# LordLiang/DrawingSpinUp

Hardware: AMD Instinct MI355X
Metric: drawings/sec end-to-end (512x512, 6 views, 24 frames) (higher is better)
Workload: dtype f16 (diffusion) / f16 table + f32 MLP (NSR) / f32 (stage-1 deformable convolutions, IS-Net, contour) / f32 with bf16 x 3 products (stage-2 convolutions; the reference: cuDNN TF32)

## Files before the change

drawingspinup_amd/csrc/mesh_decimate_gpu.hip:

```cpp
#include "common.h"

#include <math.h>
#include <stdint.h>

#include <hipcub/hipcub.hpp>

namespace {

struct D3 {
  double x, y, z;
};
__device__ inline D3 operator+(D3 a, D3 b) { return {a.x + b.x, a.y + b.y, a.z + b.z}; }
__device__ inline D3 operator-(D3 a, D3 b) { return {a.x - b.x, a.y - b.y, a.z - b.z}; }
__device__ inline D3 operator*(D3 a, double s) { return {a.x * s, a.y * s, a.z * s}; }
__device__ inline double dot3(D3 a, D3 b) { return a.x * b.x + a.y * b.y + a.z * b.z; }
__device__ inline D3 cross3(D3 a, D3 b) {
  return {a.y * b.z - a.z * b.y, a.z * b.x - a.x * b.z, a.x * b.y - a.y * b.x};
}
__device__ inline double norm3(D3 a) { return sqrt(dot3(a, a)); }

struct Quad {
  double q[10];
};
__device__ inline void quad_zero(Quad& a) {
  for (int i = 0; i < 10; ++i) a.q[i] = 0.0;
}
__device__ inline void quad_add_plane(Quad& a, D3 n, double d, double w) {
  a.q[0] += w * n.x * n.x; a.q[1] += w * n.x * n.y; a.q[2] += w * n.x * n.z;
  a.q[3] += w * n.y * n.y; a.q[4] += w * n.y * n.z; a.q[5] += w * n.z * n.z;
  a.q[6] += w * n.x * d; a.q[7] += w * n.y * d; a.q[8] += w * n.z * d;
  a.q[9] += w * d * d;
}
__device__ inline double quad_eval(const Quad& a, D3 v) {
  return v.x * (a.q[0] * v.x + 2 * a.q[1] * v.y + 2 * a.q[2] * v.z) +
         v.y * (a.q[3] * v.y + 2 * a.q[4] * v.z) + a.q[5] * v.z * v.z +
         2 * (a.q[6] * v.x + a.q[7] * v.y + a.q[8] * v.z) + a.q[9];
}
struct Row4 {
  double c[4];
};
__device__ inline void row_swap_if(Row4& a, Row4& b, bool s) {
  if (s) { const Row4 t = a; a = b; b = t; }
}
__device__ inline void row_eliminate(Row4& r, const Row4& piv, int col) {
  const double f = r.c[col] / piv.c[col];
  for (int k = 0; k < 4; ++k) r.c[k] -= f * piv.c[k];
}
__device__ inline bool quad_minimum(const Quad& a, D3 o, D3& out) {
  const double a00 = a.q[0], a01 = a.q[1], a02 = a.q[2], a11 = a.q[3], a12 = a.q[4], a22 = a.q[5];
  const double b0 = a.q[6], b1 = a.q[7], b2 = a.q[8];
  const double c00 = a11 * a22 - a12 * a12, c01 = a02 * a12 - a01 * a22, c02 = a01 * a12 - a02 * a11;
  const double det = a00 * c00 + a01 * c01 + a02 * c02;
  const double tr = a00 + a11 + a22;
  if (!(tr > 0.0) || !(fabs(det) > 1e-9 * tr * tr * tr)) return false;
  Row4 r0 = {{a00, a01, a02, -(b0 + (a00 * o.x + a01 * o.y + a02 * o.z))}};
  Row4 r1 = {{a01, a11, a12, -(b1 + (a01 * o.x + a11 * o.y + a12 * o.z))}};
  Row4 r2 = {{a02, a12, a22, -(b2 + (a02 * o.x + a12 * o.y + a22 * o.z))}};
  row_swap_if(r0, r1, fabs(r1.c[0]) > fabs(r0.c[0]));
  row_swap_if(r0, r2, fabs(r2.c[0]) > fabs(r0.c[0]));
  if (!(fabs(r0.c[0]) > 0.0)) return false;
  row_eliminate(r1, r0, 0);
  row_eliminate(r2, r0, 0);
  row_swap_if(r1, r2, fabs(r2.c[1]) > fabs(r1.c[1]));
  if (!(fabs(r1.c[1]) > 0.0)) return false;
  row_eliminate(r2, r1, 1);
  if (!(fabs(r2.c[2]) > 0.0)) return false;
  const double z = r2.c[3] / r2.c[2];
  const double y = (r1.c[3] - r1.c[2] * z) / r1.c[1];
  const double x = (r0.c[3] - r0.c[1] * y - r0.c[2] * z) / r0.c[0];
  out = {o.x + x, o.y + y, o.z + z};
  return true;
}

struct Mesh {
  double* P;
  double* Q;
  int32_t* F;
  int32_t* voff;
  int32_t* vfaces;
  int64_t nv, nf;
};

__device__ inline D3 ldP(const Mesh& m, int32_t v) { return {m.P[3 * v], m.P[3 * v + 1], m.P[3 * v + 2]}; }
__device__ inline Quad ldQ(const Mesh& m, int32_t v) {
  Quad a;
  for (int i = 0; i < 10; ++i) a.q[i] = m.Q[10 * (int64_t)v + i];
  return a;
}
__device__ inline bool tri_has(const Mesh& m, int32_t t, int32_t v) {
  return m.F[3 * t] == v || m.F[3 * t + 1] == v || m.F[3 * t + 2] == v;
}

__device__ inline void edge_target(const Mesh& m, int32_t v0, int32_t v1, double& cost, D3& vbar) {
  Quad q = ldQ(m, v0);
  const Quad q1 = ldQ(m, v1);
  for (int i = 0; i < 10; ++i) q.q[i] += q1.q[i];
  const D3 p0 = ldP(m, v0), p1 = ldP(m, v1);
  const D3 mid = (p0 + p1) * 0.5;
  if (quad_minimum(q, mid, vbar)) {
    const double len = norm3(p1 - p0);
    if (norm3(vbar - mid) <= 4.0 * len) {
      cost = quad_eval(q, vbar);
      return;
    }
  }
  const D3 cand[3] = {p0, p1, (p0 + p1) * 0.5};
  cost = quad_eval(q, cand[0]);
  vbar = cand[0];
  for (int i = 1; i < 3; ++i) {
    const double c = quad_eval(q, cand[i]);
    if (c < cost) { cost = c; vbar = cand[i]; }
  }
}

__global__ void flag_nondegenerate_kernel(const int32_t* F, int64_t nf, uint8_t* flag) {
  for (int64_t t = blockIdx.x * (int64_t)blockDim.x + threadIdx.x; t < nf; t += (int64_t)gridDim.x * blockDim.x) {
    const int32_t a = F[3 * t], b = F[3 * t + 1], c = F[3 * t + 2];
    flag[t] = (a != b && b != c && a != c) ? 1 : 0;
  }
}

__global__ void degree_kernel(const int32_t* F, int64_t nf, int32_t* deg) {
  for (int64_t i = blockIdx.x * (int64_t)blockDim.x + threadIdx.x; i < 3 * nf; i += (int64_t)gridDim.x * blockDim.x)
    atomicAdd(&deg[F[i]], 1);
}

__global__ void fill_kernel(const int32_t* F, int64_t nf, const int32_t* voff, int32_t* cursor, int32_t* vfaces) {
  for (int64_t i = blockIdx.x * (int64_t)blockDim.x + threadIdx.x; i < 3 * nf; i += (int64_t)gridDim.x * blockDim.x) {
    const int32_t v = F[i];
    vfaces[voff[v] + atomicAdd(&cursor[v], 1)] = (int32_t)(i / 3);
  }
}

__global__ void sort_lists_kernel(const int32_t* voff, int32_t* vfaces, int64_t nv) {
  for (int64_t v = blockIdx.x * (int64_t)blockDim.x + threadIdx.x; v < nv; v += (int64_t)gridDim.x * blockDim.x) {
    const int32_t b = voff[v], e = voff[v + 1];
    for (int32_t i = b + 1; i < e; ++i) {
      const int32_t x = vfaces[i];
      int32_t j = i - 1;
      while (j >= b && vfaces[j] > x) { vfaces[j + 1] = vfaces[j]; --j; }
      vfaces[j + 1] = x;
    }
  }
}

__device__ inline bool has_half_edge(const Mesh& m, int32_t a, int32_t b) {
  for (int32_t i = m.voff[a]; i < m.voff[a + 1]; ++i) {
    const int32_t t = m.vfaces[i];
    for (int k = 0; k < 3; ++k)
      if (m.F[3 * t + k] == a && m.F[3 * t + (k + 1) % 3] == b) return true;
  }
  return false;
}

__global__ void init_quadrics_kernel(Mesh m, double boundary_weight) {
  for (int64_t v = blockIdx.x * (int64_t)blockDim.x + threadIdx.x; v < m.nv; v += (int64_t)gridDim.x * blockDim.x) {
    Quad q;
    quad_zero(q);
    for (int32_t i = m.voff[v]; i < m.voff[v + 1]; ++i) {
      const int32_t t = m.vfaces[i];
      const int32_t a = m.F[3 * t], b = m.F[3 * t + 1], c = m.F[3 * t + 2];
      const D3 pa = ldP(m, a), pb = ldP(m, b), pc = ldP(m, c);
      const D3 cr = cross3(pb - pa, pc - pa);
      const double l = norm3(cr);
      if (!(l > 0.0)) continue;
      const D3 n = cr * (1.0 / l);
      quad_add_plane(q, n, -dot3(n, pa), 0.5 * l);
      if (boundary_weight > 0.0) {
        for (int k = 0; k < 3; ++k) {
          const int32_t e0 = m.F[3 * t + k], e1 = m.F[3 * t + (k + 1) % 3];
          if (e0 != (int32_t)v && e1 != (int32_t)v) continue;
          if (has_half_edge(m, e1, e0)) continue;
          int same = 0;
          for (int32_t j = m.voff[e0]; j < m.voff[e0 + 1]; ++j) {
            const int32_t t2 = m.vfaces[j];
            for (int kk = 0; kk < 3; ++kk)
              if (m.F[3 * t2 + kk] == e0 && m.F[3 * t2 + (kk + 1) % 3] == e1) ++same;
          }
          if (same != 1) continue;
          const int32_t lo = e0 < e1 ? e0 : e1, hi = e0 < e1 ? e1 : e0;
          D3 en = cross3(ldP(m, hi) - ldP(m, lo), n);
          const double el = norm3(en);
          if (!(el > 0.0)) continue;
          en = en * (1.0 / el);
          quad_add_plane(q, en, -dot3(en, ldP(m, lo)), boundary_weight * 0.5 * l);
        }
      }
    }
    for (int i = 0; i < 10; ++i) m.Q[10 * v + i] = q.q[i];
  }
}

__global__ void owner_flags_kernel(Mesh m, uint8_t* flag) {
  for (int64_t i = blockIdx.x * (int64_t)blockDim.x + threadIdx.x; i < 3 * m.nf; i += (int64_t)gridDim.x * blockDim.x) {
    const int64_t t = i / 3;
    const int k = (int)(i % 3);
    const int32_t a = m.F[3 * t + k], b = m.F[3 * t + (k + 1) % 3];
    flag[i] = (a < b || (a > b && !has_half_edge(m, b, a))) ? 1 : 0;
  }
}

typedef unsigned long long Reject;

__device__ inline unsigned long long ekey(int32_t a, int32_t b) {
  const uint32_t lo = a < b ? a : b, hi = a < b ? b : a;
  return ((unsigned long long)lo << 32) | hi;
}
__device__ inline unsigned long long mix64(unsigned long long k) {
  k ^= k >> 33; k *= 0xff51afd7ed558ccdull; k ^= k >> 33; k *= 0xc4ceb9fe1a85ec53ull; k ^= k >> 33;
  return k;
}
__device__ inline uint32_t slot_of(unsigned long long key, uint32_t n_slots) {
  return (uint32_t)(mix64(key) % n_slots);
}
__device__ inline unsigned long long reject_tag(unsigned long long key, uint32_t ver0, uint32_t ver1) {
  return mix64(key ^ mix64(((unsigned long long)ver0 << 32) | ver1)) & 0xffffffffffffull;
}

__global__ void edge_cost_kernel(Mesh m, const int32_t* edges, int64_t ne, const Reject* rej, uint32_t n_slots,
                                 const uint32_t* vver, uint32_t* cost_bits, uint32_t* edge_idx) {
  for (int64_t e = blockIdx.x * (int64_t)blockDim.x + threadIdx.x; e < ne; e += (int64_t)gridDim.x * blockDim.x) {
    const int32_t h = edges[e];
    const int32_t t = h / 3, k = h % 3;
    const int32_t a = m.F[3 * t + k], b = m.F[3 * t + (k + 1) % 3];
    const int32_t v0 = a < b ? a : b, v1 = a < b ? b : a;
    double cost; D3 vb;
    edge_target(m, v0, v1, cost, vb);
    float c = (float)(cost > 0.0 ? cost : 0.0);
    const unsigned long long key = ekey(v0, v1);
    if ((rej[slot_of(key, n_slots)] & 0xffffffffffffull) == reject_tag(key, vver[v0], vver[v1])) c = INFINITY;
    cost_bits[e] = __float_as_uint(c);
    edge_idx[e] = (uint32_t)e;
  }
}

__device__ inline void edge_ends(const Mesh& m, int32_t h, int32_t& v0, int32_t& v1) {
  const int32_t t = h / 3, k = h % 3;
  const int32_t a = m.F[3 * t + k], b = m.F[3 * t + (k + 1) % 3];
  v0 = a < b ? a : b;
  v1 = a < b ? b : a;
}

__device__ inline unsigned long long priority_of(int32_t v0, int32_t v1, uint32_t round, uint32_t r) {
  unsigned long long k = ekey(v0, v1) ^ ((unsigned long long)round * 0x9e3779b97f4a7c15ull);
  k ^= k >> 31; k *= 0xbf58476d1ce4e5b9ull; k ^= k >> 29; k *= 0x94d049bb133111ebull; k ^= k >> 32;
  return (k << 32) | r;
}

__device__ inline bool is_dirty(const Mesh& m, int32_t v0, int32_t v1, const uint32_t* touched, uint32_t round) {
  for (int pass = 0; pass < 2; ++pass) {
    const int32_t v = pass ? v1 : v0;
    for (int32_t i = m.voff[v]; i < m.voff[v + 1]; ++i) {
      const int32_t t = m.vfaces[i];
      for (int k = 0; k < 3; ++k)
        if (touched[m.F[3 * t + k]] == round) return true;
    }
  }
  return touched[v0] == round || touched[v1] == round;
}

__global__ void claim_kernel(Mesh m, const int32_t* edges, const uint32_t* sorted_idx, const uint32_t* sorted_cost,
                             int64_t ncand, uint32_t round, uint32_t seed, const uint32_t* touched,
                             const Reject* rej, uint32_t n_slots, const uint32_t* vver,
                             unsigned long long* claim) {
  for (int64_t r = blockIdx.x * (int64_t)blockDim.x + threadIdx.x; r < ncand; r += (int64_t)gridDim.x * blockDim.x) {
    if (sorted_cost[r] == 0x7f800000u) continue;
    int32_t v0, v1;
    edge_ends(m, edges[sorted_idx[r]], v0, v1);
    if (is_dirty(m, v0, v1, touched, round)) continue;
    {
      const unsigned long long key = ekey(v0, v1);
      if ((rej[slot_of(key, n_slots)] & 0xffffffffffffull) == reject_tag(key, vver[v0], vver[v1])) continue;
    }
    const unsigned long long pr = priority_of(v0, v1, seed, (uint32_t)r);
    for (int pass = 0; pass < 2; ++pass) {
      const int32_t v = pass ? v1 : v0;
      for (int32_t i = m.voff[v]; i < m.voff[v + 1]; ++i) {
        const int32_t t = m.vfaces[i];
        for (int k = 0; k < 3; ++k) atomicMin(&claim[m.F[3 * t + k]], pr);
      }
    }
  }
}

__global__ void collapse_kernel(Mesh m, const int32_t* edges, const uint32_t* sorted_idx, const uint32_t* sorted_cost,
                                int64_t ncand, uint32_t round, uint32_t seed, const unsigned long long* claim,
                                int link_test, uint8_t* f_alive, Reject* rej, uint32_t n_slots, uint32_t* vver,
                                uint32_t* touched_next, const uint32_t* touched, int32_t* counters) {
  for (int64_t r = blockIdx.x * (int64_t)blockDim.x + threadIdx.x; r < ncand; r += (int64_t)gridDim.x * blockDim.x) {
    if (sorted_cost[r] == 0x7f800000u) continue;
    int32_t v0, v1;
    edge_ends(m, edges[sorted_idx[r]], v0, v1);
    const unsigned long long pr = priority_of(v0, v1, seed, (uint32_t)r);
    if (claim[v0] != pr || claim[v1] != pr) continue;
    if (is_dirty(m, v0, v1, touched, round)) continue;
    double cost; D3 vbar;
    edge_target(m, v0, v1, cost, vbar);
    const int32_t b0 = m.voff[v0], e0 = m.voff[v0 + 1], b1 = m.voff[v1], e1 = m.voff[v1 + 1];
    int shared = 0;
    bool bad = false;
    for (int pass = 0; pass < 2 && !bad; ++pass) {
      const int32_t mv = pass ? v0 : v1, other = pass ? v1 : v0;
      for (int32_t i = m.voff[mv]; i < m.voff[mv + 1]; ++i) {
        const int32_t t = m.vfaces[i];
        if (tri_has(m, t, other)) { if (!pass) ++shared; continue; }
        D3 p[3], q[3];
        for (int k = 0; k < 3; ++k) {
          p[k] = ldP(m, m.F[3 * t + k]);
          q[k] = m.F[3 * t + k] == mv ? vbar : p[k];
        }
        const D3 before = cross3(p[1] - p[0], p[2] - p[0]);
        const D3 after = cross3(q[1] - q[0], q[2] - q[0]);
        if (dot3(before, after) < 0.0) { bad = true; break; }
      }
    }
    if (!bad && shared == 0) bad = true;
    if (!bad && link_test) {
      int common = 0;
      for (int32_t i = b0; i < e0; ++i) {
        const int32_t t = m.vfaces[i];
        for (int k = 0; k < 3; ++k) {
          const int32_t u = m.F[3 * t + k];
          if (u == v0 || u == v1) continue;
          bool first = true;
          for (int32_t j = b0; j < i && first; ++j)
            if (tri_has(m, m.vfaces[j], u)) first = false;
          if (first)
            for (int kk = 0; kk < k; ++kk)
              if (m.F[3 * t + kk] == u) first = false;
          if (!first) continue;
          bool in1 = false;
          for (int32_t j = b1; j < e1 && !in1; ++j)
            if (tri_has(m, m.vfaces[j], u)) in1 = true;
          if (in1) ++common;
        }
      }
      if (common != shared) bad = true;
      for (int32_t j = b1; j < e1 && !bad; ++j) {
        const int32_t t1 = m.vfaces[j];
        if (tri_has(m, t1, v0)) continue;
        int32_t xy[2], k2 = 0;
        for (int k = 0; k < 3; ++k)
          if (m.F[3 * t1 + k] != v1 && k2 < 2) xy[k2++] = m.F[3 * t1 + k];
        if (k2 < 2) continue;
        for (int32_t i = b0; i < e0; ++i) {
          const int32_t t0 = m.vfaces[i];
          if (!tri_has(m, t0, v1) && tri_has(m, t0, xy[0]) && tri_has(m, t0, xy[1])) { bad = true; break; }
        }
      }
    }
    if (bad) {
      const unsigned long long key = ekey(v0, v1);
      atomicMax(&rej[slot_of(key, n_slots)],
                ((unsigned long long)(round & 0xffffu) << 48) | reject_tag(key, vver[v0], vver[v1]));
      atomicAdd(&counters[1], 1);
      continue;
    }
    for (int pass = 0; pass < 2; ++pass) {
      const int32_t v = pass ? v1 : v0;
      for (int32_t i = m.voff[v]; i < m.voff[v + 1]; ++i) {
        const int32_t t = m.vfaces[i];
        for (int k = 0; k < 3; ++k) atomicAdd(&vver[m.F[3 * t + k]], 1u);
      }
    }
    int removed = 0;
    for (int32_t j = b1; j < e1; ++j) {
      const int32_t t = m.vfaces[j];
      if (tri_has(m, t, v0)) {
        f_alive[t] = 0;
        ++removed;
      } else {
        for (int k = 0; k < 3; ++k)
          if (m.F[3 * t + k] == v1) m.F[3 * t + k] = v0;
      }
    }
    m.P[3 * v0] = vbar.x; m.P[3 * v0 + 1] = vbar.y; m.P[3 * v0 + 2] = vbar.z;
    for (int i = 0; i < 10; ++i) m.Q[10 * (int64_t)v0 + i] += m.Q[10 * (int64_t)v1 + i];
    touched_next[v0] = round;
    touched_next[v1] = round;
    atomicAdd(&counters[0], 1);
    atomicAdd(&counters[2], removed);
  }
}

struct Tri {
  int32_t a, b, c;
};

inline size_t align256(size_t x) { return (x + 255) & ~(size_t)255; }

struct Layout {
  size_t off_Q, off_F2, off_voff, off_cursor, off_vfaces, off_flag, off_edges, off_iota, off_cost, off_cost2,
      off_idx, off_idx2, off_claim, off_vver, off_touched, off_touched2, off_rej, off_counters, off_nsel, off_cub, cub_bytes, total;
  uint32_t n_slots;
};

Layout make_layout(int64_t nv, int64_t nf) {
  Layout L;
  size_t o = 0;
  auto take = [&](size_t bytes) { size_t r = o; o += align256(bytes); return r; };
  L.off_Q = take((size_t)nv * 10 * sizeof(double));
  L.off_F2 = take((size_t)nf * 3 * sizeof(int32_t));
  L.off_voff = take((size_t)(nv + 1) * sizeof(int32_t));
  L.off_cursor = take((size_t)(nv + 1) * sizeof(int32_t));
  L.off_vfaces = take((size_t)nf * 3 * sizeof(int32_t));
  L.off_flag = take((size_t)nf * 3);
  L.off_edges = take((size_t)nf * 3 * sizeof(int32_t));
  L.off_iota = take((size_t)nf * 3 * sizeof(int32_t));
  L.off_cost = take((size_t)nf * 3 * sizeof(uint32_t));
  L.off_cost2 = take((size_t)nf * 3 * sizeof(uint32_t));
  L.off_idx = take((size_t)nf * 3 * sizeof(uint32_t));
  L.off_idx2 = take((size_t)nf * 3 * sizeof(uint32_t));
  L.off_claim = take((size_t)nv * sizeof(unsigned long long));
  L.off_vver = take((size_t)nv * sizeof(uint32_t));
  L.off_touched = take((size_t)nv * sizeof(uint32_t));
  L.off_touched2 = take((size_t)nv * sizeof(uint32_t));
  L.n_slots = (uint32_t)(nv * 2 + 1024);
  L.off_rej = take((size_t)L.n_slots * sizeof(Reject));
  L.off_counters = take(64);
  L.off_nsel = take(64);
  size_t b_scan = 0, b_sel_i = 0, b_sel_t = 0, b_sort = 0;
  hipcub::DeviceScan::ExclusiveSum(nullptr, b_scan, (int32_t*)nullptr, (int32_t*)nullptr, (int)(nv + 1));
  hipcub::DeviceSelect::Flagged(nullptr, b_sel_i, (int32_t*)nullptr, (uint8_t*)nullptr, (int32_t*)nullptr,
                                (int32_t*)nullptr, (int)(3 * nf));
  hipcub::DeviceSelect::Flagged(nullptr, b_sel_t, (Tri*)nullptr, (uint8_t*)nullptr, (Tri*)nullptr, (int32_t*)nullptr,
                                (int)nf);
  hipcub::DeviceRadixSort::SortPairs(nullptr, b_sort, (uint32_t*)nullptr, (uint32_t*)nullptr, (uint32_t*)nullptr,
                                     (uint32_t*)nullptr, (int)(3 * nf));
  L.cub_bytes = std::max(std::max(b_scan, b_sel_i), std::max(b_sel_t, b_sort)) + 256;
  L.off_cub = take(L.cub_bytes);
  L.total = o;
  return L;
}

__global__ void iota_kernel(int32_t* p, int64_t n) {
  for (int64_t i = blockIdx.x * (int64_t)blockDim.x + threadIdx.x; i < n; i += (int64_t)gridDim.x * blockDim.x) p[i] = (int32_t)i;
}

}

#define DSU_HIP_TRY(expr)                       \
  do {                                          \
    if ((expr) != hipSuccess) return DSU_ELAUNCH; \
  } while (0)

extern "C" {

int64_t dsu_mesh_decimate_parallel_workspace_bytes(int64_t n_verts, int64_t n_faces) {
  if (n_verts < 0 || n_faces < 0 || n_verts > (1 << 30) || n_faces > (1 << 29)) return DSU_EINVAL;
  return (int64_t)make_layout(n_verts, n_faces).total;
}

int dsu_mesh_decimate_parallel(double* verts, int64_t n_verts, int32_t* faces, int64_t n_faces,
                               int64_t stop_faces, int64_t floor_faces, double boundary_weight, int32_t flags,
                               int32_t max_rounds, double* out_quadrics, int64_t* out_n_faces,
                               int32_t* out_stats, void* workspace, int64_t workspace_bytes, void* stream) {
  if (n_verts < 0 || n_faces < 0 || stop_faces < floor_faces || floor_faces < 0 || !out_n_faces ||
      (n_verts && !verts) || (n_faces && !faces) || !(boundary_weight >= 0.0) || max_rounds < 0 ||
      n_verts > (1 << 30) || n_faces > (1 << 29))
    return DSU_EINVAL;
  hipStream_t s = (hipStream_t)stream;
  if (out_stats) out_stats[0] = out_stats[1] = out_stats[2] = 0;
  *out_n_faces = n_faces;
  if (n_faces == 0 || n_verts == 0) return DSU_OK;
  const Layout L = make_layout(n_verts, n_faces);
  if (!workspace || workspace_bytes < (int64_t)L.total) return DSU_EINVAL;
  char* w = (char*)workspace;
  double* Q = (double*)(w + L.off_Q);
  int32_t* F2 = (int32_t*)(w + L.off_F2);
  int32_t* voff = (int32_t*)(w + L.off_voff);
  int32_t* cursor = (int32_t*)(w + L.off_cursor);
  int32_t* vfaces = (int32_t*)(w + L.off_vfaces);
  uint8_t* flag = (uint8_t*)(w + L.off_flag);
  int32_t* edges = (int32_t*)(w + L.off_edges);
  int32_t* iota = (int32_t*)(w + L.off_iota);
  uint32_t* cost = (uint32_t*)(w + L.off_cost);
  uint32_t* cost2 = (uint32_t*)(w + L.off_cost2);
  uint32_t* idx = (uint32_t*)(w + L.off_idx);
  uint32_t* idx2 = (uint32_t*)(w + L.off_idx2);
  unsigned long long* claim = (unsigned long long*)(w + L.off_claim);
  uint32_t* vver = (uint32_t*)(w + L.off_vver);
  uint32_t* touched = (uint32_t*)(w + L.off_touched);
  uint32_t* touched2 = (uint32_t*)(w + L.off_touched2);
  Reject* rej = (Reject*)(w + L.off_rej);
  int32_t* counters = (int32_t*)(w + L.off_counters);
  int32_t* nsel = (int32_t*)(w + L.off_nsel);
  void* cub = (void*)(w + L.off_cub);
  const int T = 256;
  const int PASSES = 4;
  const int link_test = !(flags & 1);

  int32_t* F = faces;
  int64_t nf = n_faces;
  int32_t host_n = 0;
  auto compact_faces = [&]() -> int {
    size_t b = L.cub_bytes;
    if (hipcub::DeviceSelect::Flagged(cub, b, (Tri*)F, flag, (Tri*)F2, nsel, (int)nf, s) != hipSuccess)
      return DSU_ELAUNCH;
    if (hipMemcpyAsync(&host_n, nsel, sizeof(int32_t), hipMemcpyDeviceToHost, s) != hipSuccess) return DSU_ELAUNCH;
    if (hipStreamSynchronize(s) != hipSuccess) return DSU_ELAUNCH;
    nf = host_n;
    if (nf && hipMemcpyAsync(F, F2, (size_t)nf * 3 * sizeof(int32_t), hipMemcpyDeviceToDevice, s) != hipSuccess)
      return DSU_ELAUNCH;
    return DSU_OK;
  };
  auto build_csr = [&]() -> int {
    DSU_HIP_TRY(hipMemsetAsync(cursor, 0, (size_t)(n_verts + 1) * sizeof(int32_t), s));
    degree_kernel<<<dsu_capped_blocks(3 * nf, T), T, 0, s>>>(F, nf, cursor);
    size_t b = L.cub_bytes;
    if (hipcub::DeviceScan::ExclusiveSum(cub, b, cursor, voff, (int)(n_verts + 1), s) != hipSuccess)
      return DSU_ELAUNCH;
    DSU_HIP_TRY(hipMemsetAsync(cursor, 0, (size_t)(n_verts + 1) * sizeof(int32_t), s));
    fill_kernel<<<dsu_capped_blocks(3 * nf, T), T, 0, s>>>(F, nf, voff, cursor, vfaces);
    sort_lists_kernel<<<dsu_capped_blocks(n_verts, T), T, 0, s>>>(voff, vfaces, n_verts);
    DSU_CHECK_LAUNCH();
    return DSU_OK;
  };

  flag_nondegenerate_kernel<<<dsu_capped_blocks(nf, T), T, 0, s>>>(F, nf, flag);
  DSU_CHECK_LAUNCH();
  int rc = compact_faces();
  if (rc) return rc;
  DSU_HIP_TRY(hipMemsetAsync(vver, 0, (size_t)n_verts * sizeof(uint32_t), s));
  DSU_HIP_TRY(hipMemsetAsync(touched, 0xff, (size_t)n_verts * sizeof(uint32_t), s));
  DSU_HIP_TRY(hipMemsetAsync(touched2, 0xff, (size_t)n_verts * sizeof(uint32_t), s));
  DSU_HIP_TRY(hipMemsetAsync(rej, 0, (size_t)L.n_slots * sizeof(Reject), s));
  iota_kernel<<<dsu_capped_blocks(3 * nf, T), T, 0, s>>>(iota, 3 * nf);
  if ((rc = build_csr())) return rc;
  Mesh m{verts, Q, F, voff, vfaces, n_verts, nf};
  init_quadrics_kernel<<<dsu_capped_blocks(n_verts, T), T, 0, s>>>(m, boundary_weight);
  DSU_CHECK_LAUNCH();

  int rounds = 0, applied_total = 0, rejected_total = 0, stall = 0;
  while (nf > stop_faces && rounds < max_rounds) {
    const int64_t budget = (nf - floor_faces) / 2;
    if (budget < 1) break;
    m.nf = nf;
    owner_flags_kernel<<<dsu_capped_blocks(3 * nf, T), T, 0, s>>>(m, flag);
    DSU_CHECK_LAUNCH();
    size_t b = L.cub_bytes;
    if (hipcub::DeviceSelect::Flagged(cub, b, iota, flag, edges, nsel, (int)(3 * nf), s) != hipSuccess)
      return DSU_ELAUNCH;
    DSU_HIP_TRY(hipMemcpyAsync(&host_n, nsel, sizeof(int32_t), hipMemcpyDeviceToHost, s));
    DSU_HIP_TRY(hipStreamSynchronize(s));
    const int64_t ne = host_n;
    if (ne == 0) break;
    edge_cost_kernel<<<dsu_capped_blocks(ne, T), T, 0, s>>>(m, edges, ne, rej, L.n_slots, vver, cost, idx);
    DSU_CHECK_LAUNCH();
    b = L.cub_bytes;
    if (hipcub::DeviceRadixSort::SortPairs(cub, b, cost, cost2, idx, idx2, (int)ne, 0, 32, s) != hipSuccess)
      return DSU_ELAUNCH;
    int64_t ncand = budget < ne / 2 ? budget : ne / 2;
    if (ncand < 1) ncand = 1;
    DSU_HIP_TRY(hipMemsetAsync(counters, 0, 64, s));
    DSU_HIP_TRY(hipMemsetAsync(flag, 1, (size_t)nf, s));
    for (int pass = 0; pass < PASSES; ++pass) {
      const uint32_t seed = (uint32_t)rounds * 16u + (uint32_t)pass;
      DSU_HIP_TRY(hipMemsetAsync(claim, 0xff, (size_t)n_verts * sizeof(unsigned long long), s));
      claim_kernel<<<dsu_capped_blocks(ncand, T), T, 0, s>>>(m, edges, idx2, cost2, ncand, (uint32_t)rounds, seed,
                                                             touched, rej, L.n_slots, vver, claim);
      collapse_kernel<<<dsu_capped_blocks(ncand, T), T, 0, s>>>(m, edges, idx2, cost2, ncand, (uint32_t)rounds, seed,
                                                                claim, link_test, flag, rej, L.n_slots, vver,
                                                                touched2, touched, counters);
      DSU_CHECK_LAUNCH();
      DSU_HIP_TRY(hipMemcpyAsync(touched, touched2, (size_t)n_verts * sizeof(uint32_t), hipMemcpyDeviceToDevice, s));
    }
    int32_t hc[3];
    DSU_HIP_TRY(hipMemcpyAsync(hc, counters, sizeof(hc), hipMemcpyDeviceToHost, s));
    DSU_HIP_TRY(hipStreamSynchronize(s));
    ++rounds;
    applied_total += hc[0];
    rejected_total += hc[1];
    if (hc[0] == 0) {
      if (++stall >= 4) break;
      continue;
    }
    stall = 0;
    const int64_t before = nf;
    if ((rc = compact_faces())) return rc;
    if ((before - nf) * 200 < before && nf <= 4 * stop_faces) break;
    if (nf == 0) break;
    if ((rc = build_csr())) return rc;
  }
  if (out_quadrics)
    DSU_HIP_TRY(hipMemcpyAsync(out_quadrics, Q, (size_t)n_verts * 10 * sizeof(double), hipMemcpyDeviceToDevice, s));
  DSU_HIP_TRY(hipStreamSynchronize(s));
  *out_n_faces = nf;
  if (out_stats) { out_stats[0] = rounds; out_stats[1] = applied_total; out_stats[2] = rejected_total; }
  return DSU_OK;
}

}
```

Measured before the change: 0.3747.

## Compact surviving edge candidates between decimation passes and cache vertex fans

The parallel edge-collapse loop now carries a compacted candidate list (wave ballot appends) from pass to pass, so later claim/collapse launches only visit edges that are still live instead of rescanning all sorted candidates. Dirty tracking switches to per-pass marks in a single touched array, which removes the touched2 buffer and the device-to-device copy after every pass. The one-ring of each endpoint is gathered into registers once and reused for both the dirty test and the claim stamps, and claim atomics are skipped when the current value is already smaller. Counters are reduced per wave before the atomics. The cost is more complex bookkeeping, reuse of the cost/idx buffers as list storage, and a small change in the order collapses happen, which can change the decimated mesh.

```diff
diff --git a/drawingspinup_amd/csrc/mesh_decimate_gpu.hip b/drawingspinup_amd/csrc/mesh_decimate_gpu.hip
--- a/drawingspinup_amd/csrc/mesh_decimate_gpu.hip
+++ b/drawingspinup_amd/csrc/mesh_decimate_gpu.hip
@@ -247,53 +247,135 @@
   return (k << 32) | r;
 }
 
-__device__ inline bool is_dirty(const Mesh& m, int32_t v0, int32_t v1, const uint32_t* touched, uint32_t round) {
-  for (int pass = 0; pass < 2; ++pass) {
-    const int32_t v = pass ? v1 : v0;
-    for (int32_t i = m.voff[v]; i < m.voff[v + 1]; ++i) {
-      const int32_t t = m.vfaces[i];
-      for (int k = 0; k < 3; ++k)
-        if (touched[m.F[3 * t + k]] == round) return true;
-    }
-  }
-  return touched[v0] == round || touched[v1] == round;
-}
-
+#define DSU_MARK_ROUND_BITS 27
+#define DSU_MARK_PASS_SLOTS 16u
+
+typedef uint4 Cand;
+
+#define DSU_FAN 8
+__device__ inline void fan_ring(const Mesh& m, int32_t v, int32_t (&u)[2 * DSU_FAN]) {
+  const int32_t b = m.voff[v], e = m.voff[v + 1];
+#pragma unroll
+  for (int j = 0; j < DSU_FAN; ++j) {
+    int32_t nx = -1, pv = -1;
+    if (b + j < e) {
+      const int32_t t = m.vfaces[b + j];
+      const int32_t a0 = m.F[3 * t], a1 = m.F[3 * t + 1], a2 = m.F[3 * t + 2];
+      if (a0 == v) { nx = a1; pv = a2; }
+      else if (a1 == v) { nx = a2; pv = a0; }
+      else { nx = a0; pv = a1; }
+    }
+    u[j] = nx;
+    u[DSU_FAN + j] = pv;
+  }
+#pragma unroll
+  for (int j = 0; j < DSU_FAN; ++j) {
+    int32_t same = 0;
+#pragma unroll
+    for (int i = 0; i < DSU_FAN; ++i) same |= (int32_t)(u[i] == u[DSU_FAN + j]);
+    u[DSU_FAN + j] = same ? -1 : u[DSU_FAN + j];
+  }
+}
+
+__device__ inline bool mark_earlier_pass(const uint32_t* touched, int32_t u, uint32_t mark_base, uint32_t pass) {
+  return touched[u] - mark_base < pass;
+}
+
+__device__ inline void stamp(unsigned long long* claim, int32_t u, unsigned long long pr) {
+  if (claim[u] > pr) atomicMin(&claim[u], pr);
+}
+
+__device__ inline void wave_append(bool keep, Cand c, Cand* out, int32_t* n_out) {
+  const unsigned long long mask = __ballot(keep);
+  if (mask == 0) return;
+  const int lane = threadIdx.x & (DSU_WAVE - 1);
+  int32_t base = 0;
+  if (lane == 0) base = atomicAdd(n_out, (int32_t)__popcll(mask));
+  base = __shfl(base, 0);
+  if (keep) out[base + __popcll(mask & ((1ull << lane) - 1ull))] = c;
+}
+
+__device__ inline int wave_sum(int x) {
+#pragma unroll
+  for (int o = DSU_WAVE / 2; o > 0; o >>= 1) x += __shfl_xor(x, o);
+  return x;
+}
+
+template <bool FIRST>
 __global__ void claim_kernel(Mesh m, const int32_t* edges, const uint32_t* sorted_idx, const uint32_t* sorted_cost,
-                             int64_t ncand, uint32_t round, uint32_t seed, const uint32_t* touched,
+                             int64_t ncand, const Cand* in, const int32_t* n_in, Cand* out, int32_t* n_out,
+                             uint32_t mark_base, uint32_t pass, uint32_t seed, const uint32_t* touched,
                              const Reject* rej, uint32_t n_slots, const uint32_t* vver,
                              unsigned long long* claim) {
-  for (int64_t r = blockIdx.x * (int64_t)blockDim.x + threadIdx.x; r < ncand; r += (int64_t)gridDim.x * blockDim.x) {
-    if (sorted_cost[r] == 0x7f800000u) continue;
-    int32_t v0, v1;
-    edge_ends(m, edges[sorted_idx[r]], v0, v1);
-    if (is_dirty(m, v0, v1, touched, round)) continue;
-    {
-      const unsigned long long key = ekey(v0, v1);
-      if ((rej[slot_of(key, n_slots)] & 0xffffffffffffull) == reject_tag(key, vver[v0], vver[v1])) continue;
-    }
-    const unsigned long long pr = priority_of(v0, v1, seed, (uint32_t)r);
-    for (int pass = 0; pass < 2; ++pass) {
-      const int32_t v = pass ? v1 : v0;
-      for (int32_t i = m.voff[v]; i < m.voff[v + 1]; ++i) {
-        const int32_t t = m.vfaces[i];
-        for (int k = 0; k < 3; ++k) atomicMin(&claim[m.F[3 * t + k]], pr);
+  const int64_t n = FIRST ? ncand : (int64_t)*n_in;
+  const int lane = threadIdx.x & (DSU_WAVE - 1);
+  for (int64_t base = blockIdx.x * (int64_t)blockDim.x + (threadIdx.x - lane); base < n;
+       base += (int64_t)gridDim.x * blockDim.x) {
+    const int64_t i = base + lane;
+    bool keep = false, remembered = false;
+    Cand c = make_uint4(0u, 0u, 0u, 0u);
+    if (i < n) {
+      int32_t v0, v1;
+      if (FIRST) {
+        keep = sorted_cost[i] != 0x7f800000u;
+        if (keep) {
+          edge_ends(m, edges[sorted_idx[i]], v0, v1);
+          c = make_uint4((uint32_t)i, (uint32_t)v0, (uint32_t)v1, 0u);
+        }
+      } else {
+        c = in[i];
+        v0 = (int32_t)c.y; v1 = (int32_t)c.z;
+        const unsigned long long key = ekey(v0, v1);
+        remembered = (rej[slot_of(key, n_slots)] & 0xffffffffffffull) == reject_tag(key, vver[v0], vver[v1]);
+        keep = true;
       }
-    }
-  }
-}
-
-__global__ void collapse_kernel(Mesh m, const int32_t* edges, const uint32_t* sorted_idx, const uint32_t* sorted_cost,
-                                int64_t ncand, uint32_t round, uint32_t seed, const unsigned long long* claim,
-                                int link_test, uint8_t* f_alive, Reject* rej, uint32_t n_slots, uint32_t* vver,
-                                uint32_t* touched_next, const uint32_t* touched, int32_t* counters) {
-  for (int64_t r = blockIdx.x * (int64_t)blockDim.x + threadIdx.x; r < ncand; r += (int64_t)gridDim.x * blockDim.x) {
-    if (sorted_cost[r] == 0x7f800000u) continue;
-    int32_t v0, v1;
-    edge_ends(m, edges[sorted_idx[r]], v0, v1);
-    const unsigned long long pr = priority_of(v0, v1, seed, (uint32_t)r);
-    if (claim[v0] != pr || claim[v1] != pr) continue;
-    if (is_dirty(m, v0, v1, touched, round)) continue;
+      if (keep && !remembered) {
+        int32_t u0[2 * DSU_FAN], u1[2 * DSU_FAN];
+        fan_ring(m, v0, u0);
+        fan_ring(m, v1, u1);
+        const int32_t t0 = m.voff[v0] + DSU_FAN, e0 = m.voff[v0 + 1];
+        const int32_t t1 = m.voff[v1] + DSU_FAN, e1 = m.voff[v1 + 1];
+        if (!FIRST) {
+          bool dirty = mark_earlier_pass(touched, v0, mark_base, pass) | mark_earlier_pass(touched, v1, mark_base, pass);
+#pragma unroll
+          for (int j = 0; j < 2 * DSU_FAN; ++j) {
+            if (u0[j] >= 0) dirty |= mark_earlier_pass(touched, u0[j], mark_base, pass);
+            if (u1[j] >= 0) dirty |= mark_earlier_pass(touched, u1[j], mark_base, pass);
+          }
+          for (int32_t q = t0; q < e0; ++q)
+            for (int k = 0; k < 3; ++k) dirty |= mark_earlier_pass(touched, m.F[3 * m.vfaces[q] + k], mark_base, pass);
+          for (int32_t q = t1; q < e1; ++q)
+            for (int k = 0; k < 3; ++k) dirty |= mark_earlier_pass(touched, m.F[3 * m.vfaces[q] + k], mark_base, pass);
+          keep = !dirty;
+        }
+        if (keep) {
+          const unsigned long long pr = priority_of(v0, v1, seed, c.x);
+          stamp(claim, v0, pr);
+          stamp(claim, v1, pr);
+#pragma unroll
+          for (int j = 0; j < 2 * DSU_FAN; ++j) {
+            if (u0[j] >= 0 && u0[j] != v1) stamp(claim, u0[j], pr);
+            if (u1[j] >= 0 && u1[j] != v0) stamp(claim, u1[j], pr);
+          }
+          for (int32_t q = t0; q < e0; ++q)
+            for (int k = 0; k < 3; ++k) stamp(claim, m.F[3 * m.vfaces[q] + k], pr);
+          for (int32_t q = t1; q < e1; ++q)
+            for (int k = 0; k < 3; ++k) stamp(claim, m.F[3 * m.vfaces[q] + k], pr);
+        }
+      }
+    }
+    wave_append(keep, c, out, n_out);
+  }
+}
+
+struct Outcome {
+  int what;
+  int removed;
+};
+__device__ inline Outcome test_and_apply(const Mesh& m, int32_t v0, int32_t v1, uint32_t round, int link_test,
+                                     uint8_t* f_alive, Reject* rej, uint32_t n_slots, uint32_t* vver,
+                                     uint32_t* touched, uint32_t mark) {
+  {
     double cost; D3 vbar;
     edge_target(m, v0, v1, cost, vbar);
     const int32_t b0 = m.voff[v0], e0 = m.voff[v0 + 1], b1 = m.voff[v1], e1 = m.voff[v1 + 1];
@@ -339,13 +421,15 @@
       for (int32_t j = b1; j < e1 && !bad; ++j) {
         const int32_t t1 = m.vfaces[j];
         if (tri_has(m, t1, v0)) continue;
-        int32_t xy[2], k2 = 0;
-        for (int k = 0; k < 3; ++k)
-          if (m.F[3 * t1 + k] != v1 && k2 < 2) xy[k2++] = m.F[3 * t1 + k];
+        int32_t x = -1, y = -1, k2 = 0;
+        for (int k = 0; k < 3; ++k) {
+          const int32_t c = m.F[3 * t1 + k];
+          if (c != v1 && k2 < 2) { if (k2 == 0) x = c; else y = c; ++k2; }
+        }
         if (k2 < 2) continue;
         for (int32_t i = b0; i < e0; ++i) {
           const int32_t t0 = m.vfaces[i];
-          if (!tri_has(m, t0, v1) && tri_has(m, t0, xy[0]) && tri_has(m, t0, xy[1])) { bad = true; break; }
+          if (!tri_has(m, t0, v1) && tri_has(m, t0, x) && tri_has(m, t0, y)) { bad = true; break; }
         }
       }
     }
@@ -353,8 +437,7 @@
       const unsigned long long key = ekey(v0, v1);
       atomicMax(&rej[slot_of(key, n_slots)],
                 ((unsigned long long)(round & 0xffffu) << 48) | reject_tag(key, vver[v0], vver[v1]));
-      atomicAdd(&counters[1], 1);
-      continue;
+      return {1, 0};
     }
     for (int pass = 0; pass < 2; ++pass) {
       const int32_t v = pass ? v1 : v0;
@@ -376,10 +459,46 @@
     }
     m.P[3 * v0] = vbar.x; m.P[3 * v0 + 1] = vbar.y; m.P[3 * v0 + 2] = vbar.z;
     for (int i = 0; i < 10; ++i) m.Q[10 * (int64_t)v0 + i] += m.Q[10 * (int64_t)v1 + i];
-    touched_next[v0] = round;
-    touched_next[v1] = round;
-    atomicAdd(&counters[0], 1);
-    atomicAdd(&counters[2], removed);
+    touched[v0] = mark;
+    touched[v1] = mark;
+    return {2, removed};
+  }
+}
+
+__global__ void collapse_kernel(Mesh m, const Cand* in, const int32_t* n_in, Cand* out, int32_t* n_out,
+                                uint32_t round, uint32_t mark, uint32_t seed, const unsigned long long* claim,
+                                int link_test, uint8_t* f_alive, Reject* rej, uint32_t n_slots, uint32_t* vver,
+                                uint32_t* touched, int32_t* counters) {
+  const int32_t n = *n_in;
+  const int lane = threadIdx.x & (DSU_WAVE - 1);
+  const int32_t waves = (int32_t)(gridDim.x * (blockDim.x / DSU_WAVE));
+  const int32_t wave = (int32_t)(blockIdx.x * (blockDim.x / DSU_WAVE) + threadIdx.x / DSU_WAVE);
+  const int32_t per_wave = (n + waves - 1) / waves;
+  const int32_t end = (wave + 1) * per_wave < n ? (wave + 1) * per_wave : n;
+  int n_applied = 0, n_rejected = 0, n_removed = 0;
+  for (int32_t base = wave * per_wave; base < end; base += DSU_WAVE) {
+    const int32_t i = base + lane;
+    Outcome o = {0, 0};
+    bool stay = false;
+    Cand c = make_uint4(0u, 0u, 0u, 0u);
+    if (i < end) {
+      c = in[i];
+      const int32_t v0 = (int32_t)c.y, v1 = (int32_t)c.z;
+      const unsigned long long pr = priority_of(v0, v1, seed, c.x);
+      if (claim[v0] == pr && claim[v1] == pr)
+        o = test_and_apply(m, v0, v1, round, link_test, f_alive, rej, n_slots, vver, touched, mark);
+      stay = o.what != 2;
+    }
+    const int applied = (int)__popcll(__ballot(o.what == 2));
+    n_applied += applied;
+    n_rejected += (int)__popcll(__ballot(o.what == 1));
+    if (applied) n_removed += wave_sum(o.removed);
+    if (out) wave_append(stay, c, out, n_out);
+  }
+  if (lane == 0) {
+    if (n_applied) atomicAdd(&counters[0], n_applied);
+    if (n_rejected) atomicAdd(&counters[1], n_rejected);
+    if (n_removed) atomicAdd(&counters[2], n_removed);
   }
 }
 
@@ -391,7 +510,7 @@
 
 struct Layout {
   size_t off_Q, off_F2, off_voff, off_cursor, off_vfaces, off_flag, off_edges, off_iota, off_cost, off_cost2,
-      off_idx, off_idx2, off_claim, off_vver, off_touched, off_touched2, off_rej, off_counters, off_nsel, off_cub, cub_bytes, total;
+      off_idx, off_idx2, off_claim, off_vver, off_touched, off_rej, off_counters, off_nsel, off_cub, cub_bytes, total;
   uint32_t n_slots;
 };
 
@@ -414,7 +533,6 @@
   L.off_claim = take((size_t)nv * sizeof(unsigned long long));
   L.off_vver = take((size_t)nv * sizeof(uint32_t));
   L.off_touched = take((size_t)nv * sizeof(uint32_t));
-  L.off_touched2 = take((size_t)nv * sizeof(uint32_t));
   L.n_slots = (uint32_t)(nv * 2 + 1024);
   L.off_rej = take((size_t)L.n_slots * sizeof(Reject));
   L.off_counters = take(64);
@@ -481,13 +599,15 @@
   unsigned long long* claim = (unsigned long long*)(w + L.off_claim);
   uint32_t* vver = (uint32_t*)(w + L.off_vver);
   uint32_t* touched = (uint32_t*)(w + L.off_touched);
-  uint32_t* touched2 = (uint32_t*)(w + L.off_touched2);
   Reject* rej = (Reject*)(w + L.off_rej);
   int32_t* counters = (int32_t*)(w + L.off_counters);
   int32_t* nsel = (int32_t*)(w + L.off_nsel);
   void* cub = (void*)(w + L.off_cub);
   const int T = 256;
   const int PASSES = 4;
+  static_assert(PASSES <= (int)DSU_MARK_PASS_SLOTS && 4 + 2 * PASSES <= 16, "marks and list counts of a round");
+  Cand* list_a = (Cand*)cost;
+  Cand* list_b = (Cand*)idx;
   const int link_test = !(flags & 1);
 
   int32_t* F = faces;
@@ -523,7 +643,6 @@
   if (rc) return rc;
   DSU_HIP_TRY(hipMemsetAsync(vver, 0, (size_t)n_verts * sizeof(uint32_t), s));
   DSU_HIP_TRY(hipMemsetAsync(touched, 0xff, (size_t)n_verts * sizeof(uint32_t), s));
-  DSU_HIP_TRY(hipMemsetAsync(touched2, 0xff, (size_t)n_verts * sizeof(uint32_t), s));
   DSU_HIP_TRY(hipMemsetAsync(rej, 0, (size_t)L.n_slots * sizeof(Reject), s));
   iota_kernel<<<dsu_capped_blocks(3 * nf, T), T, 0, s>>>(iota, 3 * nf);
   if ((rc = build_csr())) return rc;
@@ -554,16 +673,27 @@
     if (ncand < 1) ncand = 1;
     DSU_HIP_TRY(hipMemsetAsync(counters, 0, 64, s));
     DSU_HIP_TRY(hipMemsetAsync(flag, 1, (size_t)nf, s));
+    const uint32_t mark_round = (uint32_t)rounds & ((1u << DSU_MARK_ROUND_BITS) - 1u);
+    if (rounds > 0 && mark_round == 0)
+      DSU_HIP_TRY(hipMemsetAsync(touched, 0xff, (size_t)n_verts * sizeof(uint32_t), s));
+    const uint32_t mark_base = mark_round * DSU_MARK_PASS_SLOTS;
+    const int blocks = dsu_capped_blocks(ncand, T);
     for (int pass = 0; pass < PASSES; ++pass) {
       const uint32_t seed = (uint32_t)rounds * 16u + (uint32_t)pass;
+      int32_t* n_claimed = counters + 4 + 2 * pass;
+      int32_t* n_left = counters + 5 + 2 * pass;
       DSU_HIP_TRY(hipMemsetAsync(claim, 0xff, (size_t)n_verts * sizeof(unsigned long long), s));
-      claim_kernel<<<dsu_capped_blocks(ncand, T), T, 0, s>>>(m, edges, idx2, cost2, ncand, (uint32_t)rounds, seed,
-                                                             touched, rej, L.n_slots, vver, claim);
-      collapse_kernel<<<dsu_capped_blocks(ncand, T), T, 0, s>>>(m, edges, idx2, cost2, ncand, (uint32_t)rounds, seed,
-                                                                claim, link_test, flag, rej, L.n_slots, vver,
-                                                                touched2, touched, counters);
+      if (pass == 0)
+        claim_kernel<true><<<blocks, T, 0, s>>>(m, edges, idx2, cost2, ncand, nullptr, nullptr, list_b, n_claimed,
+                                                mark_base, 0u, seed, touched, rej, L.n_slots, vver, claim);
+      else
+        claim_kernel<false><<<blocks, T, 0, s>>>(m, edges, idx2, cost2, ncand, list_a, n_left - 2, list_b, n_claimed,
+                                                 mark_base, (uint32_t)pass, seed, touched, rej, L.n_slots, vver,
+                                                 claim);
+      collapse_kernel<<<blocks, T, 0, s>>>(m, list_b, n_claimed, pass + 1 < PASSES ? list_a : nullptr, n_left,
+                                           (uint32_t)rounds, mark_base + (uint32_t)pass, seed, claim, link_test, flag,
+                                           rej, L.n_slots, vver, touched, counters);
       DSU_CHECK_LAUNCH();
-      DSU_HIP_TRY(hipMemcpyAsync(touched, touched2, (size_t)n_verts * sizeof(uint32_t), hipMemcpyDeviceToDevice, s));
     }
     int32_t hc[3];
     DSU_HIP_TRY(hipMemcpyAsync(hc, counters, sizeof(hc), hipMemcpyDeviceToHost, s));
```

After: 0.3820 (median of 6 runs). 2.0% higher.
